# nemochina2008/soundgen_beta

Hardware: AMD Instinct MI355X
Metric: synthesized audio samples/sec (whole node) @44.1 kHz; RMS error vs R ref (higher is better)
Workload: dtype fp32 (fp64 phase); 1 GPU; C5: 65536 soundgen() calls drawn from the 33 presets (mixed sylLen and pitch contours), 44.1 kHz; calls=65536, calls_rank0=65536, samples=4311979595, parallelism=dp1 (one batch split by calls, LPT), plans_per_rank=6, failed_calls=0

## Files before the change

soundgen_beta_amd/csrc/sg_dev.h:

```cpp
#pragma once
#include <stdint.h>

struct SgSeg {
  double t0;
  double c0, c1, c2, c3, c4;
};

struct SgEpoch {
  int64_t w_off;
  int64_t amp_off;
  int64_t knot_off;
  int32_t seg_off;
  int32_t nseg;
  int32_t n;
  int32_t G;
  int32_t R;
  int32_t u0;
  double x1, xG;
  double xby;
  double invD;
  int32_t dj0, dj1;
  int64_t dk0;
  int32_t syl;
  int32_t pad;
// ... 131 lines not shown
  int32_t wl, M, nstages, fb;
  int32_t radix[SG_FFT_MAX_STAGES];
  int64_t tw;
  int64_t win;
  int32_t lds_bytes;
  int32_t kind;
  uint32_t mr_magic[SG_FFT_MAX_STAGES], ns_magic[SG_FFT_MAX_STAGES];
  uint32_t m_magic, hp_magic;
  int64_t tws;
};

constexpr int SG_FFT_WG = 0;
constexpr int SG_FFT_WAVE = 1;
constexpr int SG_FFT_DFT = 2;
constexpr int SG_FFT_ODD = 3;
constexpr int SG_WAVE_STATE = 24;
constexpr int SG_FFT_WAVES = 8;

#ifndef SG_NOISE_WAVES
#define SG_NOISE_WAVES 12
#endif
constexpr int SG_FFT_WAVES_NOISE = SG_NOISE_WAVES;
constexpr int sg_fft_waves(int phase) { return phase == 0 ? SG_FFT_WAVES_NOISE : SG_FFT_WAVES; }
constexpr int SG_PF_SRC = 20;
constexpr int SG_PF_PAIR = 10;

constexpr int SG_FRAME_FILTER = 0;
constexpr int SG_FRAME_NOISE = 1;
struct SgFrame {
  int64_t src;
// ... 156 lines not shown
```

soundgen_beta_amd/csrc/sg_exec.cpp:

```cpp
#include "sg_exec.h"
#include "sg_amp.h"
#include "sg_prof.h"

#include <algorithm>
#include <chrono>
#include <exception>
#include <thread>
#include <cmath>
#include <climits>
#include <atomic>
#include <map>
#include <cstdlib>
#include <cstdio>
#include <cstring>
#include <string>

namespace sg {

namespace {
#define HIPCHK(x)                                                                         \
  do {                                                                                    \
    hipError_t _e = (x);                                                                  \
    if (_e != hipSuccess)                                                                 \
      throw SgError(SG_E_DEVICE, std::string(#x) + ": " + hipGetErrorString(_e));     \
// ... 784 lines not shown
  DevicePlan& D0 = *runs[0].D;
  HIPCHK(hipEventRecord(D0.ev_fork, s));
  HIPCHK(hipStreamWaitEvent(s2, D0.ev_fork, 0));
  for (const PlanRun& r : runs) {
    device_execute_harm(*r.B, *r.D, r.out, s2, nullptr);
    HIPCHK(hipEventRecord(r.D->ev_join, s2));
  }
  for (const PlanRun& r : runs) device_execute_spec(*r.B, *r.D, r.out, s, nullptr, true, r.D->ev_join);
  HIPCHK(hipGetLastError());
}

void device_execute_spec(const Batch& B, const DevicePlan& D, float* d_out, hipStream_t s,
                         std::vector<SgProfEvent>* prof, bool join, hipEvent_t harm_done) {
  launch_spec_env(D, B, s);
  auto phase = [&](int ph) {
    const int64_t* r = B.fgroup_range[ph];
    const int64_t nseg = B.seg_range[ph][1] - B.seg_range[ph][0];
    hipEvent_t e0 = nullptr, e1 = nullptr;
    if (prof && nseg > 0) {
      HIPCHK(hipEventCreate(&e0));
      HIPCHK(hipEventCreate(&e1));
      HIPCHK(hipEventRecord(e0, s));
    }
    launch_stft_ola(D, ph, B.seg_range[ph][0], nseg, B.fgroup_lds[ph][0], s);
    if (prof && nseg > 0) {
      HIPCHK(hipEventRecord(e1, s));
      prof->push_back({SG_PROF_STFT_OLA, e0, e1});
    }
    launch_fft_frames(D, r[1], r[2] - r[1], B.fgroup_lds[ph][1], s);
    launch_fft_frames64(D, B, ph, s);
    const int64_t t0 = ph == 0 ? 0 : B.olatile_split, t1 = ph == 0 ? B.olatile_split : (int64_t)B.olatiles.size();
    const int64_t o0 = ph == 0 ? 0 : B.ola_split, o1 = ph == 0 ? B.ola_split : (int64_t)B.olas_dev.size();
    launch_ola(D, t0, t1 - t0, s);
    launch_ola_max(D, o0, o1 - o0, s);
  };
  phase(0);
  for (const Batch::Copy& c : B.copies)
    HIPCHK(hipMemcpyAsync(D.fs + c.fs_off, D.fl + c.fl_off, (size_t)c.n * sizeof(float), hipMemcpyDeviceToDevice, s));
  if (join) HIPCHK(hipStreamWaitEvent(s, harm_done, 0));
  launch_mix(D, 0, B.mixtile_hp, d_out, s);
  launch_mix_hp(D, B.mixtile_hp, B.mixtile_split - B.mixtile_hp, s);
  phase(1);
  launch_mix(D, B.mixtile_split, (int64_t)B.mixtiles.size() - B.mixtile_split, d_out, s);
  HIPCHK(hipGetLastError());
// ... 4 lines not shown
```

soundgen_beta_amd/csrc/sg_exec.h:

```cpp
#pragma once
#include <hip/hip_runtime.h>

#include <utility>
#include <vector>

#include "sg_plan.h"

namespace sg {

struct PcmJob {
  char* buf = nullptr;
  SgPcmCall* calls = nullptr;
  SgPcmTile* tiles = nullptr;
  SgPcmStat* stats = nullptr;
  int64_t n = 0, ntiles = 0;
  void prepare(const int64_t* off, const int64_t* len, int64_t n_calls, hipStream_t s);
  void run(const void* in, bool f64, int mode, double nrange, int16_t* out, hipStream_t s) const;
  void free();
};

struct DevicePlan {
  bool uploaded = false;
  char* arena = nullptr;
  size_t arena_bytes = 0;
// ... 88 lines not shown
void launch_ugather(const SgUJob* jobs, int64_t n_jobs, const float* us, float* fl, hipStream_t s);
void launch_sine_bank(const DevicePlan& D, int64_t k0, int64_t n, hipStream_t s);
void launch_sine_bank_pairs(const DevicePlan& D, int64_t k0, int64_t n, hipStream_t s);
void launch_sine_bank_tall(const DevicePlan& D, int64_t k0, int64_t n, hipStream_t s);
void launch_sine_bank_tall_pairs(const DevicePlan& D, int64_t k0, int64_t n, hipStream_t s);
void launch_syl_max(const DevicePlan& D, int64_t s0, int64_t n_syls, hipStream_t s);
void launch_piece_max(const DevicePlan& D, int64_t p0, int64_t n_ptiles, hipStream_t s);
void launch_harm_finalize(const DevicePlan& D, int64_t f0, int64_t n_stiles, float* out, hipStream_t s);
void launch_harm_copy(const DevicePlan& D, int64_t c0, int64_t n_ctiles, float* out, hipStream_t s);
void launch_sine_bank_hp(const DevicePlan& D, int64_t n, hipStream_t s);
void launch_sine_bank_tab(const DevicePlan& D, int logn, int64_t j0, int64_t n, float* out, hipStream_t s);
void launch_piece_max_hp(const DevicePlan& D, int64_t p0, int64_t n_ptiles, hipStream_t s);
void launch_harm_finalize_hp(const DevicePlan& D, int64_t n_stiles, hipStream_t s);
void launch_mix_hp(const DevicePlan& D, int64_t t0, int64_t n_tiles, hipStream_t s);
void launch_fft_frames64(const DevicePlan& D, const Batch& B, int ph, hipStream_t s);
void launch_fft_frames(const DevicePlan& D, int64_t g0, int64_t n_groups, int lds_bytes, hipStream_t s);
void launch_stft_ola(const DevicePlan& D, int phase, int64_t s0, int64_t n_segs, int lds_bytes, hipStream_t s);
void launch_ola(const DevicePlan& D, int64_t t0, int64_t n_tiles, hipStream_t s);
void launch_ola_max(const DevicePlan& D, int64_t o0, int64_t n_olas, hipStream_t s);
void launch_fft_probe(const SgFftGeom* geom, const float* fl, float* data, int M, int nframes, int inverse,
                      hipStream_t s);
void launch_mix(const DevicePlan& D, int64_t t0, int64_t n_tiles, float* out, hipStream_t s);
void launch_spec_env(const DevicePlan& D, const Batch& B, hipStream_t s);

}
```

soundgen_beta_amd/csrc/sg_fft.hip:

```cpp
#include <hip/hip_runtime.h>

#include <type_traits>

#include "sg_dev.h"
#include "sg_devfn.h"
#include "sg_fft64_dev.h"
#include "sg_roots.h"

namespace {

typedef float v2 __attribute__((ext_vector_type(2)));
__device__ __forceinline__ v2 V(float2 a) { return v2{a.x, a.y}; }
__device__ __forceinline__ float2 F(v2 a) { return make_float2(a.x, a.y); }
__device__ __forceinline__ v2 pfma(v2 a, v2 b, v2 c) { return __builtin_elementwise_fma(a, b, c); }
__device__ __forceinline__ v2 splat(float c) { return v2{c, c}; }
__device__ __forceinline__ v2 vmul(v2 a, v2 w) {
  v2 t, r;
  __asm__("v_pk_mul_f32 %0, %1, %2 op_sel_hi:[0,1]" : "=v"(t) : "v"(a), "v"(w));
  __asm__("v_pk_fma_f32 %0, %1, %2, %3 op_sel:[1,1,0] op_sel_hi:[1,0,1] neg_lo:[0,1,0]"
          : "=v"(r) : "v"(a), "v"(w), "v"(t));
  return r;
}
__device__ __forceinline__ v2 vmulc(v2 a, v2 w) {
  v2 t, r;
// ... 91 lines not shown
};

__device__ __forceinline__ void pack_pair(float2 yk, float2 ymk, float2 wNk, float2& zk, float2& zmk) {
  const float2 e = cadd(yk, cconj(ymk));
  const float2 d = csub(yk, cconj(ymk));
  const float2 o = cmulc(d, wNk);
  zk = make_float2(e.x - o.y, e.y + o.x);
  const float2 e2 = cadd(ymk, cconj(yk));
  const float2 d2 = csub(ymk, cconj(yk));
  const float2 o2 = make_float2(-(d2.x * wNk.x - d2.y * wNk.y), -(d2.x * wNk.y + d2.y * wNk.x));
  zmk = make_float2(e2.x - o2.y, e2.y + o2.x);
}

constexpr int SG_FFT_THREADS = 512;
constexpr int SG_FFT_SLOTS = 8192;

template <int R>
struct NbOf {
  static constexpr int value = (SG_FFT_SLOTS / SG_FFT_THREADS + R - 1) / R;
};

__device__ __forceinline__ int udiv(int n, uint32_t magic) {
  return magic ? (int)__umulhi((uint32_t)n, magic) : n;
}

template <int R, bool INV>
__device__ __forceinline__ void stage_ip(float2* X, int M, int Ns, const float2* twS, int fb, uint32_t mr_magic,
                                         uint32_t ns_magic) {
  constexpr int NB = NbOf<R>::value;
  constexpr bool ODD = (R % 2) == 1;
  constexpr int H = ODD ? (R - 1) / 2 : 1;
  const int MR = M / R;
  const int total = fb * MR;
  v2 st[NB][R];
  int base_o[NB];
  bool live[NB];
#pragma unroll
  for (int q = 0; q < NB; ++q) {
    const int idx = threadIdx.x + q * SG_FFT_THREADS;
    live[q] = idx < total;
    base_o[q] = 0;
    if (!live[q]) continue;
    const int f = udiv(idx, mr_magic);
    const int j = idx - f * MR;
    const float2* x = X + f * M;
    float2 v[R];
#pragma unroll
    for (int r = 0; r < R; ++r) v[r] = x[j + r * MR];
    const int jm = j - udiv(j, ns_magic) * Ns;
    if (Ns > 1) {
      const float2* tw = twS + (Ns - 1) + jm;
#pragma unroll
      for (int r = 1; r < R; ++r) {
        const float2 w = tw[(r - 1) * Ns];
// ... 27 lines not shown
#pragma unroll
      for (int k = 1; k <= H; ++k) {
        v2 a, b;
        odd_out<R, INV>(st[q], k, a, b);
        y[k * Ns] = F(a);
        y[(R - k) * Ns] = F(b);
      }
    } else {
#pragma unroll
      for (int r = 0; r < R; ++r) y[r * Ns] = F(st[q][r]);
    }
  }
  __syncthreads();
}

template <bool INV>
__device__ void fft_ip(float2* X, const SgFftGeom& g, const float2* twS, int fb) {
  int Ns = 1;
  for (int s = 0; s < g.nstages; ++s) {
    const int R = g.radix[s];
    const uint32_t mm = g.mr_magic[s], nm = g.ns_magic[s];
    int Ms = g.M;
    Ms = __builtin_amdgcn_readfirstlane(Ms);
    switch (R) {
#define SG_STAGE(RR) \
      case RR: stage_ip<RR, INV>(X, Ms, Ns, twS, fb, mm, nm); break;
      SG_STAGE(2) SG_STAGE(3) SG_STAGE(4) SG_STAGE(5) SG_STAGE(7) SG_STAGE(11) SG_STAGE(13) SG_STAGE(17)
      SG_STAGE(19) SG_STAGE(23) SG_STAGE(29) SG_STAGE(31)
#undef SG_STAGE
      default: break;
    }
    Ns *= R;
  }
}

__device__ __forceinline__ void sg_wave_fence() { __asm__ __volatile__("" ::: "memory"); }

template <int R>
struct NbW {
  static constexpr int value = SG_WAVE_STATE / R > 0 ? SG_WAVE_STATE / R : 1;
};
// ... 227 lines not shown
  }
  sg_wave_fence();
}

template <bool INV, int CM, int R0, int R1, int R2, bool MFMA = true, bool LAST = true>
__device__ __forceinline__ void fft_wc(float2* X, const float2* twS, const float4* A29, int lane SG_ST_PARAMS) {
  if constexpr (MFMA && CM == 1102 && R0 == 29) stage29_mfma<INV>(X, A29, lane);
  else stage_w<R0, INV, CM, 1>(X, CM, 1, twS, 0u, lane);
  SG_ST(INV ? 5 : 1);
  stage_w<R1, INV, CM, R0>(X, CM, R0, twS, 0u, lane);
  SG_ST(INV ? 6 : 2);
  if constexpr (LAST) stage_w<R2, INV, CM, R0 * R1>(X, CM, R0 * R1, twS, 0u, lane);
  SG_ST(INV ? 7 : 3);
}

template <bool INV>
__device__ void cdft(float2* X, const SgCdft& c, const SgFftGeom* __restrict__ geoms, const float* __restrict__ fl,
                     float2* Z, float2* tw) {
  const SgFftGeom& gs = geoms[c.geom];
  const int T = c.L ? c.L : c.n;
  const float2* twg = reinterpret_cast<const float2*>(fl + gs.tws);
  for (int t = threadIdx.x; t < T - 1; t += SG_FFT_THREADS) tw[t] = twg[t];
  if (!c.L) {
    __syncthreads();
    fft_ip<INV>(X, gs, tw, 1);
    return;
  }
  const int n = c.n, L = c.L;
  const float2* ch = reinterpret_cast<const float2*>(fl + c.chirp);
  const float2* bf = reinterpret_cast<const float2*>(fl + c.bf);
  for (int j = threadIdx.x; j < L; j += SG_FFT_THREADS)
    Z[j] = j < n ? cmul(INV ? cconj(X[j]) : X[j], ch[j]) : make_float2(0.f, 0.f);
  __syncthreads();
  fft_ip<false>(Z, gs, tw, 1);
  for (int k = threadIdx.x; k < L; k += SG_FFT_THREADS) Z[k] = cmul(Z[k], bf[k]);
  __syncthreads();
  fft_ip<true>(Z, gs, tw, 1);
  for (int k = threadIdx.x; k < n; k += SG_FFT_THREADS) {
    const float2 v = cmul(Z[k], ch[k]);
    X[k] = INV ? cconj(v) : v;
  }
  __syncthreads();
}

__device__ void odd_frame(const SgFrameGroup& G, const SgFrame* __restrict__ frames, const SgFftGeom& g,
                          const SgFftGeom* __restrict__ geoms, const float* __restrict__ fl, float* __restrict__ fs,
                          float4* lds4) {
  const int N = g.wl, M = g.M, N2 = 2 * M;
  const int T = max(g.cd[0].L ? g.cd[0].L : g.cd[0].n, g.cd[1].L ? g.cd[1].L : g.cd[1].n);
  float2* B = reinterpret_cast<float2*>(lds4);
  float2* Z = B + N;
  float2* tw = Z + T;
  const SgFrame F = frames[G.f0];
  const float* ham = fl + g.win;
  const float* han = ham + N;
  if (G.mode == SG_FRAME_FILTER) {
    const float* s = fs + F.src;
    for (int n = threadIdx.x; n < N; n += SG_FFT_THREADS) B[n] = make_float2(s[n] * ham[n], 0.f);
    __syncthreads();
    cdft<false>(B, g.cd[0], geoms, fl, Z, tw);
    const float* env = fl + F.env;
    const float invN = 1.f / (float)N;
    for (int k = threadIdx.x; k < M; k += SG_FFT_THREADS) {
      const float sc = invN * env[k];
      const float2 y = make_float2(B[k].x * sc, B[k].y * sc);
      B[k] = y;
      if (k > 0) B[N2 - k] = cconj(y);
      if (k == M - 1) B[M] = make_float2(y.x, 0.f);
    }
  } else {
    const float* u = fl + F.src;
    const float* flt = fl + F.env;
    for (int k = threadIdx.x; k < M; k += SG_FFT_THREADS) {
      const float2 y = make_float2(u[k] * flt[k], 0.f);
      B[k] = y;
      if (k > 0) B[N2 - k] = y;
      if (k == M - 1) B[M] = y;
    }
  }
  __syncthreads();
  cdft<true>(B, g.cd[1], geoms, fl, Z, tw);
  const float invN2 = 1.f / (float)N2;
  float* d = fs + F.dst;
  for (int i = threadIdx.x; i < N; i += SG_FFT_THREADS) d[i] = B[i < N2 ? i : i - N2].x * invN2 * han[i];
}

}

extern "C" __global__ __launch_bounds__(SG_FFT_THREADS) void sg_fft_frames(
    const SgFrameGroup* __restrict__ groups, const SgFrame* __restrict__ frames, const SgFftGeom* __restrict__ geoms,
    const float* __restrict__ fl, float* __restrict__ fs) {
  extern __shared__ float4 lds4[];
  float2* A = reinterpret_cast<float2*>(lds4);
  __shared__ SgFrame fr[16];
  const SgFrameGroup G = groups[blockIdx.x];
  const SgFftGeom& g = geoms[G.geom];
  if (g.kind == SG_FFT_ODD) {
    odd_frame(G, frames, g, geoms, fl, fs, lds4);
    return;
  }
  const int M = g.M, N = g.wl, fb = G.nf;
  const float2* twg = reinterpret_cast<const float2*>(fl + g.tw);
  const float2* twN = twg + M;
  float2* twM = A + fb * M;
  if (g.kind != SG_FFT_DFT) {
    const float2* tsg = reinterpret_cast<const float2*>(fl + g.tws);
    for (int t = threadIdx.x; t < M - 1; t += SG_FFT_THREADS) twM[t] = tsg[t];
  }
  if (threadIdx.x < fb) fr[threadIdx.x] = frames[G.f0 + threadIdx.x];
  __syncthreads();
  const float* ham = fl + g.win;
  const float* han = ham + N;
  const float invN = 1.f / (float)N;
  const int half = M / 2;
  const int npairs = fb * (half + 1);
  constexpr int NP = SG_FFT_SLOTS / 2 / SG_FFT_THREADS + 1;
  if (G.mode == SG_FRAME_FILTER) {
    for (int idx = threadIdx.x; idx < fb * M; idx += SG_FFT_THREADS) {
      const int f = udiv(idx, g.m_magic), n = idx - f * M;
      const float* s = fs + fr[f].src;
      A[idx] = make_float2(s[2 * n] * ham[2 * n], s[2 * n + 1] * ham[2 * n + 1]);
    }
    __syncthreads();
    if (g.kind == SG_FFT_DFT) cdft<false>(A, g.cd[0], geoms, fl, twM, twM + g.cd[0].L);
    else fft_ip<false>(A, g, twM, fb);
    float2 zk[NP], zm[NP], zh[NP];
    int pk[NP], pf[NP];
#pragma unroll
    for (int q = 0; q < NP; ++q) {
      const int idx = threadIdx.x + q * SG_FFT_THREADS;
      pk[q] = -1;
      if (idx >= npairs) continue;
      const int f = udiv(idx, g.hp_magic), k = idx - f * (half + 1);
      if (k != 0 && k >= M - k) continue;
      pk[q] = k;
      pf[q] = f;
      const float2* z = A + f * M;
      const float* env = fl + fr[f].env;
      auto X_at = [&](int kk) -> float2 {
        const float2 a = z[kk], b = z[(M - kk) % M];
        const float2 e = make_float2(0.5f * (a.x + b.x), 0.5f * (a.y - b.y));
        const float2 dd = make_float2(a.x - b.x, a.y + b.y);
        const float2 o = make_float2(0.5f * dd.y, -0.5f * dd.x);
        return cadd(e, cmul(o, twN[kk]));
      };
// ... 18 lines not shown
    __syncthreads();
#pragma unroll
    for (int q = 0; q < NP; ++q) {
      if (pk[q] < 0) continue;
      float2* out = A + pf[q] * M;
      const int k = pk[q];
      out[k] = zk[q];
      if (k == 0) {
        if (M % 2 == 0) out[half] = zh[q];
      } else {
        out[M - k] = zm[q];
      }
    }
    __syncthreads();
  } else {
    for (int idx = threadIdx.x; idx < npairs; idx += SG_FFT_THREADS) {
      const int f = udiv(idx, g.hp_magic), k = idx - f * (half + 1);
      const SgFrame& F = fr[f];
      const float* u = fl + F.src;
      const float* flt = fl + F.env;
      float2* out = A + f * M;
      if (k == 0) {
        const float y0 = u[0] * flt[0], nyq = u[M - 1] * flt[M - 1];
        out[0] = make_float2(y0 + nyq, y0 - nyq);
        if (M % 2 == 0) {
          const float2 yk = make_float2(u[half] * flt[half], 0.f);
          float2 a, b;
          pack_pair(yk, yk, twN[half], a, b);
          out[half] = a;
        }
      } else if (k < M - k) {
        const float2 yk = make_float2(u[k] * flt[k], 0.f), ym = make_float2(u[M - k] * flt[M - k], 0.f);
        float2 a, b;
        pack_pair(yk, ym, twN[k], a, b);
        out[k] = a;
        out[M - k] = b;
      }
    }
    __syncthreads();
  }
  if (g.kind == SG_FFT_DFT) cdft<true>(A, g.cd[0], geoms, fl, twM, twM + g.cd[0].L);
  else fft_ip<true>(A, g, twM, fb);
  for (int idx = threadIdx.x; idx < fb * M; idx += SG_FFT_THREADS) {
    const int f = udiv(idx, g.m_magic), n = idx - f * M;
    const float2 v = A[idx];
    float* d = fs + fr[f].dst;
    d[2 * n] = v.x * invN * han[2 * n];
    d[2 * n + 1] = v.y * invN * han[2 * n + 1];
  }
}

static_assert(SG_PF_PAIR <= SG_PF_SRC, "noise filter pairs alias the sound pairs");
struct FramePf {
  float2 s[SG_PF_SRC];
  float2 a[SG_PF_PAIR];
  float xh, xh2;
  __device__ __forceinline__ float2& b(int i) { return s[i]; }
  __device__ __forceinline__ const float2& b(int i) const { return s[i]; }
};

template <bool FUSED = false>
__device__ __forceinline__ void frame_prefetch(FramePf& P, const SgFrame& F, int mode, int M,
                                               const float* __restrict__ fl, const float* __restrict__ fs, int lane) {
  const int half = M / 2;
// ... 1037 lines not shown
  } while (0)

static void lds_opt_in(const void* fn, int lds_bytes, const char* name) {
  static std::mutex mu;
  static std::map<std::pair<const void*, int>, int> done;
  int dev = 0;
  if (hipGetDevice(&dev) != hipSuccess) throw SgError(SG_E_DEVICE, std::string(name) + ": hipGetDevice failed");
  std::lock_guard<std::mutex> lk(mu);
  int& have = done[{fn, dev}];
  if (lds_bytes <= have) return;
  if (hipFuncSetAttribute(fn, hipFuncAttributeMaxDynamicSharedMemorySize, lds_bytes) != hipSuccess)
    throw SgError(SG_E_DEVICE, std::string(name) + ": dynamic LDS " + std::to_string(lds_bytes) + " B refused");
  have = lds_bytes;
}

void launch_fft_frames(const DevicePlan& D, int64_t g0, int64_t n_groups, int lds_bytes, hipStream_t s) {
  if (n_groups <= 0) return;
  lds_opt_in(reinterpret_cast<const void*>(&sg_fft_frames), lds_bytes, "sg_fft_frames");
  hipLaunchKernelGGL(sg_fft_frames, dim3((unsigned)n_groups), dim3(SG_FFT_THREADS), lds_bytes, s, D.fgroups + g0,
                     D.frames,
                     D.geoms, D.fl, D.fs);
  SG_LAUNCHED("sg_fft_frames");
}
void launch_stft_ola(const DevicePlan& D, int phase, int64_t s0, int64_t n_segs, int lds_bytes, hipStream_t s) {
  if (n_segs <= 0) return;
  auto* k = phase == 0 ? &sg_stft_ola_noise : &sg_stft_ola;
  lds_opt_in(reinterpret_cast<const void*>(k), lds_bytes, phase == 0 ? "sg_stft_ola_noise" : "sg_stft_ola");
  const int W = sg_fft_waves(phase);
  if (n_segs % W) throw SgError(SG_E_DEVICE, "sg_stft_ola: segment count not a multiple of the workgroup's waves");
  hipLaunchKernelGGL(k, dim3((unsigned)(n_segs / W)), dim3(W * 64), lds_bytes, s,
                     D.olasegs + s0,
                     D.olas, D.frames, D.geoms, D.fl, D.fs, D.olatilemax);
// ... 74 lines not shown
```

soundgen_beta_amd/csrc/sg_plan.h:

```cpp
#pragma once
#include <cstdint>
#include <functional>
#include <memory>
#include <utility>
#include <vector>

#include "sg_dev.h"
#include "sg_rmath.h"
#include "soundgen_hip.h"

namespace sg {

template <class T>
struct NoInitAlloc : std::allocator<T> {
  template <class U>
  struct rebind { using other = NoInitAlloc<U>; };
  NoInitAlloc() = default;
  template <class U>
  NoInitAlloc(const NoInitAlloc<U>&) noexcept {}
  T* allocate(size_t n) {
    if (n * sizeof(T) < SG_BULK_HUGE) return std::allocator<T>::allocate(n);
    return static_cast<T*>(bulk_alloc(n * sizeof(T)));
  }
  void deallocate(T* p, size_t n) noexcept {
// ... 75 lines not shown
  std::vector<SgOla> olas[2];
  std::vector<SgFrame64> frames64;
  std::vector<int32_t> roots64_wl;
  std::vector<int64_t> roots64_off, frames64_tab;
  int64_t roots64_total = 0;
  int32_t frames64_maxwl = 0;
  int64_t frames64_noise = 0;
  int64_t frames64_w[2] = {0, 0};
  std::vector<SgNoiseItem> items;
  std::vector<SgMix> mixes[2];
  struct Copy { int64_t fl_off, fs_off, n; };
  std::vector<Copy> copies;
  std::vector<SgFrameGroup> fgroups;
  int64_t fgroup_range[2][3] = {{0, 0, 0}, {0, 0, 0}};
  int fgroup_lds[2][2] = {{0, 0}, {0, 0}};
  std::vector<SgOla> olas_dev;
  std::vector<SgOlaTile> olatiles;
  int64_t olatile_split = 0, ola_split = 0;
  std::vector<SgSegment> olasegs;
  int32_t n_segslots = 0;
  int64_t seg_range[2][2] = {{0, 0}, {0, 0}};
  std::vector<SgMix> mixes_dev;
  std::vector<SgMixTile> mixtiles;
  int64_t mixtile_split = 0;
  int64_t mixtile_hp = 0;
  bulk<double> cknots;
  int64_t w_total = 0;
  int64_t w64_total = 0;
  int64_t fh_total = 0;
  int64_t hp_bouts = 0;
// ... 91 lines not shown
```

soundgen_beta_amd/csrc/sg_plan_spec.cpp:

```cpp
#include <algorithm>
#include <atomic>
#include <cmath>
#include <complex>
#include <cstdio>
#include <cstdlib>
#include <cstring>
#include <map>
#include <memory>
#include <mutex>
#include <string>

#include "sg_plan.h"
#include "sg_prof.h"

#ifndef SG_SEG_SORT
#define SG_SEG_SORT 1
#endif
#ifndef SG_ENV_SORT
#define SG_ENV_SORT 1
#endif

namespace sg {

namespace {
// ... 116 lines not shown
      if (m > 0) b[L - m] = b[m];
    }
    dft_smooth(b, bf);
    vec v(2 * (size_t)L);
    for (int k = 0; k < L; ++k) {
      v[2 * k] = bf[k].real() / L;
      v[2 * k + 1] = bf[k].imag() / L;
    }
    return v;
  });
  c.chirp = fl_push(B, ch->data(), (int64_t)ch->size());
  c.bf = fl_push(B, bv->data(), (int64_t)bv->size());
  return c;
}
static int cdft_size(const SgCdft& c) { return c.L ? c.L : c.n; }

static int geometry_odd(Batch& B, int wl) {
  SgFftGeom g{};
  g.wl = wl;
  g.M = wl / 2;
  g.kind = SG_FFT_ODD;
  g.fb = 1;
  g.cd[0] = make_cdft(B, wl);
  g.cd[1] = make_cdft(B, 2 * g.M);
  const int T = std::max(cdft_size(g.cd[0]), cdft_size(g.cd[1]));
  g.lds_bytes = (int32_t)(((int64_t)wl + 2 * (int64_t)T) * 8);
  if (g.lds_bytes > 160 * 1024) throw SgError(SG_E_UNSUPPORTED, "FFT: odd window length exceeds the LDS budget");
  g.win = push_windows(B, wl);
  for (size_t i = 0; i < B.geoms.size(); ++i)
    if (B.geoms[i].wl == wl) return (int)i;
  B.geoms.push_back(g);
  return (int)B.geoms.size() - 1;
}

int geometry(Batch& B, int wl) {
  for (size_t i = 0; i < B.geoms.size(); ++i)
    if (B.geoms[i].wl == wl) return (int)i;
// ... 51 lines not shown
    });
    g.tws = fl_push(B, ts->data(), (int64_t)ts->size());
  }
  g.win = push_windows(B, wl);
  g.kind = dft ? SG_FFT_DFT : SG_FFT_WAVE;
  for (int s = 0; s < g.nstages && !dft; ++s) {
    const int r = g.radix[s], nb = (g.M / r + 63) / 64;
    if (nb > std::max(1, SG_WAVE_STATE / r)) g.kind = SG_FFT_WG;
  }
  if (!dft && (g.M > 64 * SG_PF_SRC || g.M / 2 + 1 > 64 * SG_PF_PAIR)) g.kind = SG_FFT_WG;
  if (!dft && (int64_t)(SG_FFT_WAVES + 4) * g.M * 8 > 160 * 1024) g.kind = SG_FFT_WG;
  if (g.kind == SG_FFT_WAVE) {
    g.fb = SG_FFT_WAVES;
    g.lds_bytes = (SG_FFT_WAVES + 4) * g.M * 8;
  } else if (g.kind == SG_FFT_DFT) {
    g.fb = 1;
    g.lds_bytes = (g.M + 2 * g.cd[0].L) * 8;
    if (g.lds_bytes > 160 * 1024) throw SgError(SG_E_UNSUPPORTED, "FFT: Bluestein frame exceeds the LDS budget");
  } else {
    g.fb = std::max(1, std::min(16, kFftSlots / g.M));
    if (g.fb * g.M > kFftSlots) throw SgError(SG_E_UNSUPPORTED, "FFT: window too long for LDS (wl > 16384)");
    g.lds_bytes = (g.fb + 1) * g.M * 8;
  }
  auto magic = [](int d) -> uint32_t { return d <= 1 ? 0u : (uint32_t)(((1ull << 32) + (uint64_t)d - 1) / (uint64_t)d); };
  int ns = 1;
  for (int s = 0; s < g.nstages; ++s) {
    g.mr_magic[s] = magic(g.M / g.radix[s]);
    g.ns_magic[s] = magic(ns);
    ns *= g.radix[s];
  }
  g.m_magic = magic(g.M);
// ... 552 lines not shown
      for (size_t w = i; w < i + 4 && w < B.envtasks.size(); ++w) { mx = std::max(mx, cost(B.envtasks[w])); wsum += cost(B.envtasks[w]); }
      wmax += 4 * mx;
    }
    std::fprintf(stderr, "sg plan: envelope tasks %zu, workgroup cost %.3g, used %.3g (%.1f%% idle)\n", B.envtasks.size(), wmax,
                 wsum, wmax > 0 ? 100.0 * (wmax - wsum) / wmax : 0.0);
  }
  B.fgroups.clear();
  std::vector<int64_t> pos[2];
  for (int ph = 0; ph < 2; ++ph) {
    const size_t ng = B.geoms.size();
    std::vector<int64_t> rank(ng), start(ng + 1, 0);
    {
      std::vector<int32_t> og(ng);
      for (size_t g = 0; g < ng; ++g) og[g] = (int32_t)g;
      std::stable_sort(og.begin(), og.end(), [&](int32_t a, int32_t b) {
        const int ka = B.geoms[a].kind == SG_FFT_WAVE ? 0 : 1, kb = B.geoms[b].kind == SG_FFT_WAVE ? 0 : 1;
        return ka != kb ? ka < kb : a < b;
      });
      for (size_t r = 0; r < ng; ++r) rank[og[r]] = (int64_t)r;
    }
    for (int32_t gi : B.frame_geom[ph]) ++start[rank[gi] + 1];
    for (size_t r = 0; r < ng; ++r) start[r + 1] += start[r];
    std::vector<int64_t> idx(B.frames[ph].size());
    for (size_t i = 0; i < idx.size(); ++i) idx[start[rank[B.frame_geom[ph][i]]]++] = (int64_t)i;
    std::vector<SgFrame> fr(idx.size());
    std::vector<int32_t> fg(idx.size());
    pos[ph].assign(idx.size(), 0);
    for (size_t i = 0; i < idx.size(); ++i) {
      fr[i] = B.frames[ph][idx[i]];
      fg[i] = B.frame_geom[ph][idx[i]];
      pos[ph][idx[i]] = (int64_t)i;
    }
    B.frames[ph] = fr;
    B.frame_geom[ph] = fg;
    const int32_t base = ph == 0 ? 0 : (int32_t)B.frames[0].size();
    B.fgroup_lds[ph][0] = B.fgroup_lds[ph][1] = 0;
    B.fgroup_range[ph][0] = B.fgroup_range[ph][1] = (int64_t)B.fgroups.size();
    for (size_t i = 0; i < fr.size();) {
      const int gi = fg[i];
      const SgFftGeom& g = B.geoms[gi];
      if (g.kind == SG_FFT_WAVE) {
        B.fgroup_lds[ph][0] = std::max(B.fgroup_lds[ph][0], (sg_fft_waves(ph) + 4) * g.M * 8 + (g.M == 1102 ? 2048 : 0));
        ++i;
        continue;
      }
      size_t j = i;
      while (j < fr.size() && fg[j] == gi && (int)(j - i) < g.fb) ++j;
      B.fgroups.push_back(SgFrameGroup{gi, ph == 0 ? SG_FRAME_NOISE : SG_FRAME_FILTER, base + (int32_t)i,
                                       (int32_t)(j - i)});
      B.fgroup_lds[ph][1] = std::max(B.fgroup_lds[ph][1], g.lds_bytes);
      i = j;
    }
    B.fgroup_range[ph][2] = (int64_t)B.fgroups.size();
  }
  B.olas_dev.clear();
  B.olatiles.clear();
  B.olasegs.clear();
  B.ola_split = (int64_t)B.olas[0].size();
  for (int ph = 0; ph < 2; ++ph) {
    if (ph == 1) B.olatile_split = (int64_t)B.olatiles.size();
    const int32_t base = ph == 0 ? 0 : (int32_t)B.frames[0].size();
    for (const SgOla& o0 : B.olas[ph]) {
      SgOla o = o0;
      if (o0.fidx >= 0) o.fidx = base + (int32_t)pos[ph][o0.fidx];
      const int32_t oi = (int32_t)B.olas_dev.size();
      if (!o.fused) {
        o.tile0 = (int32_t)B.olatiles.size();
        for (int64_t q0 = 0; q0 < o.len; q0 += SG_OLA_TILE) B.olatiles.push_back(SgOlaTile{oi, 0, q0});
// ... 143 lines not shown
      const SgFftGeom& g = B.geoms[gs[i].second];
      std::string rs;
      for (int s = 0; s < g.nstages; ++s) rs += (s ? "x" : "") + std::to_string(g.radix[s]);
      std::fprintf(stderr, "sg plan: geom wl=%d M=%d radices %s: %lld frames\n", g.wl, g.M, rs.c_str(),
                   (long long)gs[i].first);
    }
    std::map<int32_t, int64_t> gun;
    for (const SgFrameGroup& fg : B.fgroups) gun[fg.geom] += fg.nf;
    for (const auto& kv : gun) {
      const SgFftGeom& g = B.geoms[kv.first];
      std::string rs;
      for (int s = 0; s < g.nstages; ++s) rs += (s ? "x" : "") + std::to_string(g.radix[s]);
      std::fprintf(stderr, "sg plan: unfused geom wl=%d M=%d kind %d radices %s: %lld frames\n", g.wl, g.M, g.kind,
                   rs.c_str(), (long long)kv.second);
    }
    std::fprintf(stderr, "sg plan: %lld fused segments (%lld slots incl. padding), %lld frames owned, %lld computed (%.1f%% recomputed)\n",
                 (long long)real, (long long)B.olasegs.size(), (long long)owned, (long long)run,
                 owned ? 100.0 * (double)(run - owned) / (double)owned : 0.0);
  }
  for (SgNoiseItem& it : B.items)
    if (it.flags & SG_ITEM_FILTER_OLA) {
      it.ola += (int32_t)B.ola_split;
      it.flags &= ~SG_ITEM_FILTER_OLA;
    }
  B.mixes_dev.clear();
  B.mixtiles.clear();
  for (int pass = 0; pass < 3; ++pass) {
    const int ph = pass == 2 ? 1 : 0;
    if (pass == 1) B.mixtile_hp = (int64_t)B.mixtiles.size();
    if (pass == 2) B.mixtile_split = (int64_t)B.mixtiles.size();
// ... 19 lines not shown
```

Before: 14.01 billion samples/s.

## Split unfused FFT frame launches into LDS size classes with a smaller-slot kernel

Unfused FFT frame groups are sorted and split into three classes by geometry kind, transform size, largest radix and LDS footprint. Bluestein and odd-length geometries that fit the smaller slot count and radix cap go to a new kernel variant. That variant is built with fewer per-thread slots, a waves-per-EU hint and only radices up to 13, and each class launches with its own LDS size. The aim is lower register and LDS pressure, so more blocks fit per CU for small frames, and less twiddle restaging through a per-geometry cache. The code also allows several sequential frames per group for DFT and odd kinds (default 1), and the extra launches add overhead.

```diff
diff --git a/soundgen_beta_amd/csrc/sg_dev.h b/soundgen_beta_amd/csrc/sg_dev.h
--- a/soundgen_beta_amd/csrc/sg_dev.h
+++ b/soundgen_beta_amd/csrc/sg_dev.h
@@ -169,6 +169,20 @@
 constexpr int SG_FFT_WAVE = 1;
 constexpr int SG_FFT_DFT = 2;
 constexpr int SG_FFT_ODD = 3;
+constexpr int SG_FRAMES_S_SLOTS = 4608;
+#ifndef SG_FRAMES_S_MAXR
+#define SG_FRAMES_S_MAXR 13
+#endif
+constexpr int SG_FRAMES_MAX_FB = 16;
+#ifndef SG_FRAMES_FB
+#define SG_FRAMES_FB 1
+#endif
+static_assert(SG_FRAMES_FB >= 1 && SG_FRAMES_FB <= SG_FRAMES_MAX_FB, "frames per group");
+#ifndef SG_FRAMES_CLASSES
+#define SG_FRAMES_CLASSES 1
+#endif
+constexpr int SG_FRAMES_NCLASS = 3;
+constexpr int SG_FRAMES_LDS_CLASS[SG_FRAMES_NCLASS - 1] = {80000, 160 * 1024};
 constexpr int SG_WAVE_STATE = 24;
 constexpr int SG_FFT_WAVES = 8;
 
diff --git a/soundgen_beta_amd/csrc/sg_exec.cpp b/soundgen_beta_amd/csrc/sg_exec.cpp
--- a/soundgen_beta_amd/csrc/sg_exec.cpp
+++ b/soundgen_beta_amd/csrc/sg_exec.cpp
@@ -822,7 +822,6 @@
                          std::vector<SgProfEvent>* prof, bool join, hipEvent_t harm_done) {
   launch_spec_env(D, B, s);
   auto phase = [&](int ph) {
-    const int64_t* r = B.fgroup_range[ph];
     const int64_t nseg = B.seg_range[ph][1] - B.seg_range[ph][0];
     hipEvent_t e0 = nullptr, e1 = nullptr;
     if (prof && nseg > 0) {
@@ -835,7 +834,9 @@
       HIPCHK(hipEventRecord(e1, s));
       prof->push_back({SG_PROF_STFT_OLA, e0, e1});
     }
-    launch_fft_frames(D, r[1], r[2] - r[1], B.fgroup_lds[ph][1], s);
+    for (int c = 0; c < SG_FRAMES_NCLASS; ++c)
+      launch_fft_frames(D, B.fgroup_cls[ph][c], B.fgroup_cls[ph][c + 1] - B.fgroup_cls[ph][c], B.fgroup_cls_lds[ph][c],
+                        c < SG_FRAMES_NCLASS - 1, s);
     launch_fft_frames64(D, B, ph, s);
     const int64_t t0 = ph == 0 ? 0 : B.olatile_split, t1 = ph == 0 ? B.olatile_split : (int64_t)B.olatiles.size();
     const int64_t o0 = ph == 0 ? 0 : B.ola_split, o1 = ph == 0 ? B.ola_split : (int64_t)B.olas_dev.size();
diff --git a/soundgen_beta_amd/csrc/sg_exec.h b/soundgen_beta_amd/csrc/sg_exec.h
--- a/soundgen_beta_amd/csrc/sg_exec.h
+++ b/soundgen_beta_amd/csrc/sg_exec.h
@@ -126,7 +126,7 @@
 void launch_harm_finalize_hp(const DevicePlan& D, int64_t n_stiles, hipStream_t s);
 void launch_mix_hp(const DevicePlan& D, int64_t t0, int64_t n_tiles, hipStream_t s);
 void launch_fft_frames64(const DevicePlan& D, const Batch& B, int ph, hipStream_t s);
-void launch_fft_frames(const DevicePlan& D, int64_t g0, int64_t n_groups, int lds_bytes, hipStream_t s);
+void launch_fft_frames(const DevicePlan& D, int64_t g0, int64_t n_groups, int lds_bytes, bool small, hipStream_t s);
 void launch_stft_ola(const DevicePlan& D, int phase, int64_t s0, int64_t n_segs, int lds_bytes, hipStream_t s);
 void launch_ola(const DevicePlan& D, int64_t t0, int64_t n_tiles, hipStream_t s);
 void launch_ola_max(const DevicePlan& D, int64_t o0, int64_t n_olas, hipStream_t s);
diff --git a/soundgen_beta_amd/csrc/sg_fft.hip b/soundgen_beta_amd/csrc/sg_fft.hip
--- a/soundgen_beta_amd/csrc/sg_fft.hip
+++ b/soundgen_beta_amd/csrc/sg_fft.hip
@@ -129,20 +129,26 @@
 
 constexpr int SG_FFT_THREADS = 512;
 constexpr int SG_FFT_SLOTS = 8192;
-
-template <int R>
+#ifndef SG_FRAMES_S_THREADS
+#define SG_FRAMES_S_THREADS 512
+#endif
+#ifndef SG_FRAMES_S_WPE
+#define SG_FRAMES_S_WPE 4
+#endif
+
+template <int R, int TH, int SL>
 struct NbOf {
-  static constexpr int value = (SG_FFT_SLOTS / SG_FFT_THREADS + R - 1) / R;
+  static constexpr int value = ((SL + TH - 1) / TH + R - 1) / R;
 };
 
 __device__ __forceinline__ int udiv(int n, uint32_t magic) {
   return magic ? (int)__umulhi((uint32_t)n, magic) : n;
 }
 
-template <int R, bool INV>
+template <int R, bool INV, int TH, int SL>
 __device__ __forceinline__ void stage_ip(float2* X, int M, int Ns, const float2* twS, int fb, uint32_t mr_magic,
                                          uint32_t ns_magic) {
-  constexpr int NB = NbOf<R>::value;
+  constexpr int NB = NbOf<R, TH, SL>::value;
   constexpr bool ODD = (R % 2) == 1;
   constexpr int H = ODD ? (R - 1) / 2 : 1;
   const int MR = M / R;
@@ -152,7 +158,7 @@
   bool live[NB];
 #pragma unroll
   for (int q = 0; q < NB; ++q) {
-    const int idx = threadIdx.x + q * SG_FFT_THREADS;
+    const int idx = threadIdx.x + q * TH;
     live[q] = idx < total;
     base_o[q] = 0;
     if (!live[q]) continue;
@@ -210,8 +216,9 @@
   __syncthreads();
 }
 
-template <bool INV>
+template <bool INV, int TH, int SL>
 __device__ void fft_ip(float2* X, const SgFftGeom& g, const float2* twS, int fb) {
+  constexpr int MAXR = SL == SG_FRAMES_S_SLOTS ? SG_FRAMES_S_MAXR : 31;
   int Ns = 1;
   for (int s = 0; s < g.nstages; ++s) {
     const int R = g.radix[s];
@@ -220,7 +227,7 @@
     Ms = __builtin_amdgcn_readfirstlane(Ms);
     switch (R) {
 #define SG_STAGE(RR) \
-      case RR: stage_ip<RR, INV>(X, Ms, Ns, twS, fb, mm, nm); break;
+      case RR: if constexpr (RR <= MAXR) stage_ip<RR, INV, TH, SL>(X, Ms, Ns, twS, fb, mm, nm); break;
       SG_STAGE(2) SG_STAGE(3) SG_STAGE(4) SG_STAGE(5) SG_STAGE(7) SG_STAGE(11) SG_STAGE(13) SG_STAGE(17)
       SG_STAGE(19) SG_STAGE(23) SG_STAGE(29) SG_STAGE(31)
 #undef SG_STAGE
@@ -478,121 +485,111 @@
   SG_ST(INV ? 7 : 3);
 }
 
-template <bool INV>
+template <bool INV, int TH, int SL>
 __device__ void cdft(float2* X, const SgCdft& c, const SgFftGeom* __restrict__ geoms, const float* __restrict__ fl,
-                     float2* Z, float2* tw) {
+                     float2* Z, float2* tw, int& staged) {
   const SgFftGeom& gs = geoms[c.geom];
   const int T = c.L ? c.L : c.n;
-  const float2* twg = reinterpret_cast<const float2*>(fl + gs.tws);
-  for (int t = threadIdx.x; t < T - 1; t += SG_FFT_THREADS) tw[t] = twg[t];
+  if (staged != c.geom) {
+    const float2* twg = reinterpret_cast<const float2*>(fl + gs.tws);
+    for (int t = threadIdx.x; t < T - 1; t += TH) tw[t] = twg[t];
+    staged = c.geom;
+  }
   if (!c.L) {
     __syncthreads();
-    fft_ip<INV>(X, gs, tw, 1);
+    fft_ip<INV, TH, SL>(X, gs, tw, 1);
     return;
   }
   const int n = c.n, L = c.L;
   const float2* ch = reinterpret_cast<const float2*>(fl + c.chirp);
   const float2* bf = reinterpret_cast<const float2*>(fl + c.bf);
-  for (int j = threadIdx.x; j < L; j += SG_FFT_THREADS)
+  for (int j = threadIdx.x; j < L; j += TH)
     Z[j] = j < n ? cmul(INV ? cconj(X[j]) : X[j], ch[j]) : make_float2(0.f, 0.f);
   __syncthreads();
-  fft_ip<false>(Z, gs, tw, 1);
-  for (int k = threadIdx.x; k < L; k += SG_FFT_THREADS) Z[k] = cmul(Z[k], bf[k]);
+  fft_ip<false, TH, SL>(Z, gs, tw, 1);
+  for (int k = threadIdx.x; k < L; k += TH) Z[k] = cmul(Z[k], bf[k]);
   __syncthreads();
-  fft_ip<true>(Z, gs, tw, 1);
-  for (int k = threadIdx.x; k < n; k += SG_FFT_THREADS) {
+  fft_ip<true, TH, SL>(Z, gs, tw, 1);
+  for (int k = threadIdx.x; k < n; k += TH) {
     const float2 v = cmul(Z[k], ch[k]);
     X[k] = INV ? cconj(v) : v;
   }
   __syncthreads();
 }
 
-__device__ void odd_frame(const SgFrameGroup& G, const SgFrame* __restrict__ frames, const SgFftGeom& g,
-                          const SgFftGeom* __restrict__ geoms, const float* __restrict__ fl, float* __restrict__ fs,
-                          float4* lds4) {
+template <int TH, int SL>
+__device__ void odd_frames(const SgFrameGroup& G, const SgFrame* __restrict__ frames, const SgFftGeom& g,
+                           const SgFftGeom* __restrict__ geoms, const float* __restrict__ fl, float* __restrict__ fs,
+                           float4* lds4) {
   const int N = g.wl, M = g.M, N2 = 2 * M;
   const int T = max(g.cd[0].L ? g.cd[0].L : g.cd[0].n, g.cd[1].L ? g.cd[1].L : g.cd[1].n);
   float2* B = reinterpret_cast<float2*>(lds4);
   float2* Z = B + N;
   float2* tw = Z + T;
-  const SgFrame F = frames[G.f0];
   const float* ham = fl + g.win;
   const float* han = ham + N;
-  if (G.mode == SG_FRAME_FILTER) {
-    const float* s = fs + F.src;
-    for (int n = threadIdx.x; n < N; n += SG_FFT_THREADS) B[n] = make_float2(s[n] * ham[n], 0.f);
+  int staged = -1;
+  for (int it = 0; it < G.nf; ++it) {
+    if (it) __syncthreads();
+    const SgFrame F = frames[G.f0 + it];
+    if (G.mode == SG_FRAME_FILTER) {
+      const float* s = fs + F.src;
+      for (int n = threadIdx.x; n < N; n += TH) B[n] = make_float2(s[n] * ham[n], 0.f);
+      __syncthreads();
+      cdft<false, TH, SL>(B, g.cd[0], geoms, fl, Z, tw, staged);
+      const float* env = fl + F.env;
+      const float invN = 1.f / (float)N;
+      for (int k = threadIdx.x; k < M; k += TH) {
+        const float sc = invN * env[k];
+        const float2 y = make_float2(B[k].x * sc, B[k].y * sc);
+        B[k] = y;
+        if (k > 0) B[N2 - k] = cconj(y);
+        if (k == M - 1) B[M] = make_float2(y.x, 0.f);
+      }
+    } else {
+      const float* u = fl + F.src;
+      const float* flt = fl + F.env;
+      for (int k = threadIdx.x; k < M; k += TH) {
+        const float2 y = make_float2(u[k] * flt[k], 0.f);
+        B[k] = y;
+        if (k > 0) B[N2 - k] = y;
+        if (k == M - 1) B[M] = y;
+      }
+    }
     __syncthreads();
-    cdft<false>(B, g.cd[0], geoms, fl, Z, tw);
-    const float* env = fl + F.env;
-    const float invN = 1.f / (float)N;
-    for (int k = threadIdx.x; k < M; k += SG_FFT_THREADS) {
-      const float sc = invN * env[k];
-      const float2 y = make_float2(B[k].x * sc, B[k].y * sc);
-      B[k] = y;
-      if (k > 0) B[N2 - k] = cconj(y);
-      if (k == M - 1) B[M] = make_float2(y.x, 0.f);
-    }
-  } else {
-    const float* u = fl + F.src;
-    const float* flt = fl + F.env;
-    for (int k = threadIdx.x; k < M; k += SG_FFT_THREADS) {
-      const float2 y = make_float2(u[k] * flt[k], 0.f);
-      B[k] = y;
-      if (k > 0) B[N2 - k] = y;
-      if (k == M - 1) B[M] = y;
-    }
-  }
-  __syncthreads();
-  cdft<true>(B, g.cd[1], geoms, fl, Z, tw);
-  const float invN2 = 1.f / (float)N2;
-  float* d = fs + F.dst;
-  for (int i = threadIdx.x; i < N; i += SG_FFT_THREADS) d[i] = B[i < N2 ? i : i - N2].x * invN2 * han[i];
-}
-
-}
-
-extern "C" __global__ __launch_bounds__(SG_FFT_THREADS) void sg_fft_frames(
-    const SgFrameGroup* __restrict__ groups, const SgFrame* __restrict__ frames, const SgFftGeom* __restrict__ geoms,
-    const float* __restrict__ fl, float* __restrict__ fs) {
-  extern __shared__ float4 lds4[];
-  float2* A = reinterpret_cast<float2*>(lds4);
-  __shared__ SgFrame fr[16];
-  const SgFrameGroup G = groups[blockIdx.x];
-  const SgFftGeom& g = geoms[G.geom];
-  if (g.kind == SG_FFT_ODD) {
-    odd_frame(G, frames, g, geoms, fl, fs, lds4);
-    return;
-  }
-  const int M = g.M, N = g.wl, fb = G.nf;
-  const float2* twg = reinterpret_cast<const float2*>(fl + g.tw);
-  const float2* twN = twg + M;
-  float2* twM = A + fb * M;
-  if (g.kind != SG_FFT_DFT) {
-    const float2* tsg = reinterpret_cast<const float2*>(fl + g.tws);
-    for (int t = threadIdx.x; t < M - 1; t += SG_FFT_THREADS) twM[t] = tsg[t];
-  }
-  if (threadIdx.x < fb) fr[threadIdx.x] = frames[G.f0 + threadIdx.x];
-  __syncthreads();
+    cdft<true, TH, SL>(B, g.cd[1], geoms, fl, Z, tw, staged);
+    const float invN2 = 1.f / (float)N2;
+    float* d = fs + F.dst;
+    for (int i = threadIdx.x; i < N; i += TH) d[i] = B[i < N2 ? i : i - N2].x * invN2 * han[i];
+  }
+}
+
+template <int TH, int SL>
+__device__ __forceinline__ void even_frames(int mode, const SgFftGeom& g, const SgFftGeom* __restrict__ geoms,
+                                            const float* __restrict__ fl, float* __restrict__ fs, float2* A,
+                                            float2* twM, const SgFrame* fr, int fb, int& staged) {
+  const int M = g.M, N = g.wl;
+  const float2* twN = reinterpret_cast<const float2*>(fl + g.tw) + M;
   const float* ham = fl + g.win;
   const float* han = ham + N;
   const float invN = 1.f / (float)N;
   const int half = M / 2;
   const int npairs = fb * (half + 1);
-  constexpr int NP = SG_FFT_SLOTS / 2 / SG_FFT_THREADS + 1;
-  if (G.mode == SG_FRAME_FILTER) {
-    for (int idx = threadIdx.x; idx < fb * M; idx += SG_FFT_THREADS) {
+  constexpr int NP = SL / 2 / TH + 1;
+  if (mode == SG_FRAME_FILTER) {
+    for (int idx = threadIdx.x; idx < fb * M; idx += TH) {
       const int f = udiv(idx, g.m_magic), n = idx - f * M;
       const float* s = fs + fr[f].src;
       A[idx] = make_float2(s[2 * n] * ham[2 * n], s[2 * n + 1] * ham[2 * n + 1]);
     }
     __syncthreads();
-    if (g.kind == SG_FFT_DFT) cdft<false>(A, g.cd[0], geoms, fl, twM, twM + g.cd[0].L);
-    else fft_ip<false>(A, g, twM, fb);
+    if (g.kind == SG_FFT_DFT) cdft<false, TH, SL>(A, g.cd[0], geoms, fl, twM, twM + g.cd[0].L, staged);
+    else fft_ip<false, TH, SL>(A, g, twM, fb);
     float2 zk[NP], zm[NP], zh[NP];
     int pk[NP], pf[NP];
 #pragma unroll
     for (int q = 0; q < NP; ++q) {
-      const int idx = threadIdx.x + q * SG_FFT_THREADS;
+      const int idx = threadIdx.x + q * TH;
       pk[q] = -1;
       if (idx >= npairs) continue;
       const int f = udiv(idx, g.hp_magic), k = idx - f * (half + 1);
@@ -641,7 +638,7 @@
     }
     __syncthreads();
   } else {
-    for (int idx = threadIdx.x; idx < npairs; idx += SG_FFT_THREADS) {
+    for (int idx = threadIdx.x; idx < npairs; idx += TH) {
       const int f = udiv(idx, g.hp_magic), k = idx - f * (half + 1);
       const SgFrame& F = fr[f];
       const float* u = fl + F.src;
@@ -666,15 +663,63 @@
     }
     __syncthreads();
   }
-  if (g.kind == SG_FFT_DFT) cdft<true>(A, g.cd[0], geoms, fl, twM, twM + g.cd[0].L);
-  else fft_ip<true>(A, g, twM, fb);
-  for (int idx = threadIdx.x; idx < fb * M; idx += SG_FFT_THREADS) {
+  if (g.kind == SG_FFT_DFT) cdft<true, TH, SL>(A, g.cd[0], geoms, fl, twM, twM + g.cd[0].L, staged);
+  else fft_ip<true, TH, SL>(A, g, twM, fb);
+  for (int idx = threadIdx.x; idx < fb * M; idx += TH) {
     const int f = udiv(idx, g.m_magic), n = idx - f * M;
     const float2 v = A[idx];
     float* d = fs + fr[f].dst;
     d[2 * n] = v.x * invN * han[2 * n];
     d[2 * n + 1] = v.y * invN * han[2 * n + 1];
   }
+}
+
+template <int TH, int SL>
+__device__ __forceinline__ void frame_group(const SgFrameGroup& G, const SgFrame* __restrict__ frames,
+                                            const SgFftGeom* __restrict__ geoms, const float* __restrict__ fl,
+                                            float* __restrict__ fs, float4* lds4, SgFrame* fr) {
+  float2* A = reinterpret_cast<float2*>(lds4);
+  const SgFftGeom& g = geoms[G.geom];
+  if (g.kind == SG_FFT_ODD) {
+    odd_frames<TH, SL>(G, frames, g, geoms, fl, fs, lds4);
+    return;
+  }
+  const int M = g.M;
+  const bool dft = g.kind == SG_FFT_DFT;
+  const int fb = dft ? 1 : G.nf;
+  float2* twM = A + fb * M;
+  if (!dft) {
+    const float2* tsg = reinterpret_cast<const float2*>(fl + g.tws);
+    for (int t = threadIdx.x; t < M - 1; t += TH) twM[t] = tsg[t];
+  }
+  if (threadIdx.x < G.nf) fr[threadIdx.x] = frames[G.f0 + threadIdx.x];
+  __syncthreads();
+  int staged = -1;
+  if (!dft) {
+    even_frames<TH, SL>(G.mode, g, geoms, fl, fs, A, twM, fr, fb, staged);
+    return;
+  }
+  for (int it = 0; it < G.nf; ++it) {
+    if (it) __syncthreads();
+    even_frames<TH, SL>(G.mode, g, geoms, fl, fs, A, twM, fr + it, 1, staged);
+  }
+}
+
+}
+
+extern "C" __global__ __launch_bounds__(SG_FFT_THREADS) void sg_fft_frames(
+    const SgFrameGroup* __restrict__ groups, const SgFrame* __restrict__ frames, const SgFftGeom* __restrict__ geoms,
+    const float* __restrict__ fl, float* __restrict__ fs) {
+  extern __shared__ float4 lds4[];
+  __shared__ SgFrame fr[SG_FRAMES_MAX_FB];
+  frame_group<SG_FFT_THREADS, SG_FFT_SLOTS>(groups[blockIdx.x], frames, geoms, fl, fs, lds4, fr);
+}
+extern "C" __global__ __launch_bounds__(SG_FRAMES_S_THREADS) __attribute__((amdgpu_waves_per_eu(SG_FRAMES_S_WPE, 8))) void
+sg_fft_frames_s(const SgFrameGroup* __restrict__ groups, const SgFrame* __restrict__ frames,
+                const SgFftGeom* __restrict__ geoms, const float* __restrict__ fl, float* __restrict__ fs) {
+  extern __shared__ float4 lds4[];
+  __shared__ SgFrame fr[SG_FRAMES_MAX_FB];
+  frame_group<SG_FRAMES_S_THREADS, SG_FRAMES_S_SLOTS>(groups[blockIdx.x], frames, geoms, fl, fs, lds4, fr);
 }
 
 static_assert(SG_PF_PAIR <= SG_PF_SRC, "noise filter pairs alias the sound pairs");
@@ -1742,8 +1787,15 @@
   have = lds_bytes;
 }
 
-void launch_fft_frames(const DevicePlan& D, int64_t g0, int64_t n_groups, int lds_bytes, hipStream_t s) {
+void launch_fft_frames(const DevicePlan& D, int64_t g0, int64_t n_groups, int lds_bytes, bool small, hipStream_t s) {
   if (n_groups <= 0) return;
+  if (small) {
+    lds_opt_in(reinterpret_cast<const void*>(&sg_fft_frames_s), lds_bytes, "sg_fft_frames_s");
+    hipLaunchKernelGGL(sg_fft_frames_s, dim3((unsigned)n_groups), dim3(SG_FRAMES_S_THREADS), lds_bytes, s,
+                       D.fgroups + g0, D.frames, D.geoms, D.fl, D.fs);
+    SG_LAUNCHED("sg_fft_frames_s");
+    return;
+  }
   lds_opt_in(reinterpret_cast<const void*>(&sg_fft_frames), lds_bytes, "sg_fft_frames");
   hipLaunchKernelGGL(sg_fft_frames, dim3((unsigned)n_groups), dim3(SG_FFT_THREADS), lds_bytes, s, D.fgroups + g0,
                      D.frames,
diff --git a/soundgen_beta_amd/csrc/sg_plan.h b/soundgen_beta_amd/csrc/sg_plan.h
--- a/soundgen_beta_amd/csrc/sg_plan.h
+++ b/soundgen_beta_amd/csrc/sg_plan.h
@@ -113,6 +113,8 @@
   std::vector<SgFrameGroup> fgroups;
   int64_t fgroup_range[2][3] = {{0, 0, 0}, {0, 0, 0}};
   int fgroup_lds[2][2] = {{0, 0}, {0, 0}};
+  int64_t fgroup_cls[2][SG_FRAMES_NCLASS + 1] = {};
+  int fgroup_cls_lds[2][SG_FRAMES_NCLASS] = {};
   std::vector<SgOla> olas_dev;
   std::vector<SgOlaTile> olatiles;
   int64_t olatile_split = 0, ola_split = 0;
diff --git a/soundgen_beta_amd/csrc/sg_plan_spec.cpp b/soundgen_beta_amd/csrc/sg_plan_spec.cpp
--- a/soundgen_beta_amd/csrc/sg_plan_spec.cpp
+++ b/soundgen_beta_amd/csrc/sg_plan_spec.cpp
@@ -154,13 +154,27 @@
   return c;
 }
 static int cdft_size(const SgCdft& c) { return c.L ? c.L : c.n; }
+constexpr int kSeqFb = SG_FRAMES_CLASSES ? SG_FRAMES_FB : 1;
+static int frames_class(const Batch& B, const SgFftGeom& g) {
+  if (!SG_FRAMES_CLASSES || (g.kind != SG_FFT_DFT && g.kind != SG_FFT_ODD)) return SG_FRAMES_NCLASS - 1;
+  const int T = g.kind == SG_FFT_DFT ? cdft_size(g.cd[0]) : std::max(cdft_size(g.cd[0]), cdft_size(g.cd[1]));
+  if (T > SG_FRAMES_S_SLOTS) return SG_FRAMES_NCLASS - 1;
+  for (int i = 0; i < (g.kind == SG_FFT_DFT ? 1 : 2); ++i) {
+    const SgFftGeom& gs = B.geoms[(size_t)g.cd[i].geom];
+    for (int s = 0; s < gs.nstages; ++s)
+      if (gs.radix[s] > SG_FRAMES_S_MAXR) return SG_FRAMES_NCLASS - 1;
+  }
+  for (int c = 0; c < SG_FRAMES_NCLASS - 1; ++c)
+    if (g.lds_bytes <= SG_FRAMES_LDS_CLASS[c]) return c;
+  return SG_FRAMES_NCLASS - 1;
+}
 
 static int geometry_odd(Batch& B, int wl) {
   SgFftGeom g{};
   g.wl = wl;
   g.M = wl / 2;
   g.kind = SG_FFT_ODD;
-  g.fb = 1;
+  g.fb = kSeqFb;
   g.cd[0] = make_cdft(B, wl);
   g.cd[1] = make_cdft(B, 2 * g.M);
   const int T = std::max(cdft_size(g.cd[0]), cdft_size(g.cd[1]));
@@ -242,7 +256,7 @@
     g.fb = SG_FFT_WAVES;
     g.lds_bytes = (SG_FFT_WAVES + 4) * g.M * 8;
   } else if (g.kind == SG_FFT_DFT) {
-    g.fb = 1;
+    g.fb = kSeqFb;
     g.lds_bytes = (g.M + 2 * g.cd[0].L) * 8;
     if (g.lds_bytes > 160 * 1024) throw SgError(SG_E_UNSUPPORTED, "FFT: Bluestein frame exceeds the LDS budget");
   } else {
@@ -825,8 +839,12 @@
       std::vector<int32_t> og(ng);
       for (size_t g = 0; g < ng; ++g) og[g] = (int32_t)g;
       std::stable_sort(og.begin(), og.end(), [&](int32_t a, int32_t b) {
-        const int ka = B.geoms[a].kind == SG_FFT_WAVE ? 0 : 1, kb = B.geoms[b].kind == SG_FFT_WAVE ? 0 : 1;
-        return ka != kb ? ka < kb : a < b;
+        const int ka = B.geoms[a].kind == SG_FFT_WAVE ? -1 : frames_class(B, B.geoms[a]);
+        const int kb = B.geoms[b].kind == SG_FFT_WAVE ? -1 : frames_class(B, B.geoms[b]);
+        if (ka != kb) return ka < kb;
+        if (SG_FRAMES_CLASSES && ka >= 0 && B.geoms[a].lds_bytes != B.geoms[b].lds_bytes)
+          return B.geoms[a].lds_bytes > B.geoms[b].lds_bytes;
+        return a < b;
       });
       for (size_t r = 0; r < ng; ++r) rank[og[r]] = (int64_t)r;
     }
@@ -847,6 +865,10 @@
     const int32_t base = ph == 0 ? 0 : (int32_t)B.frames[0].size();
     B.fgroup_lds[ph][0] = B.fgroup_lds[ph][1] = 0;
     B.fgroup_range[ph][0] = B.fgroup_range[ph][1] = (int64_t)B.fgroups.size();
+    for (int c = 0; c < SG_FRAMES_NCLASS; ++c) {
+      B.fgroup_cls[ph][c] = -1;
+      B.fgroup_cls_lds[ph][c] = 0;
+    }
     for (size_t i = 0; i < fr.size();) {
       const int gi = fg[i];
       const SgFftGeom& g = B.geoms[gi];
@@ -860,9 +882,14 @@
       B.fgroups.push_back(SgFrameGroup{gi, ph == 0 ? SG_FRAME_NOISE : SG_FRAME_FILTER, base + (int32_t)i,
                                        (int32_t)(j - i)});
       B.fgroup_lds[ph][1] = std::max(B.fgroup_lds[ph][1], g.lds_bytes);
+      const int c = frames_class(B, g);
+      if (B.fgroup_cls[ph][c] < 0) B.fgroup_cls[ph][c] = (int64_t)B.fgroups.size() - 1;
+      B.fgroup_cls_lds[ph][c] = std::max(B.fgroup_cls_lds[ph][c], g.lds_bytes);
       i = j;
     }
-    B.fgroup_range[ph][2] = (int64_t)B.fgroups.size();
+    B.fgroup_range[ph][2] = B.fgroup_cls[ph][SG_FRAMES_NCLASS] = (int64_t)B.fgroups.size();
+    for (int c = SG_FRAMES_NCLASS - 1; c >= 0; --c)
+      if (B.fgroup_cls[ph][c] < 0) B.fgroup_cls[ph][c] = B.fgroup_cls[ph][c + 1];
   }
   B.olas_dev.clear();
   B.olatiles.clear();
@@ -1036,6 +1063,28 @@
       std::fprintf(stderr, "sg plan: unfused geom wl=%d M=%d kind %d radices %s: %lld frames\n", g.wl, g.M, g.kind,
                    rs.c_str(), (long long)kv.second);
     }
+    for (int ph = 0; ph < 2; ++ph) {
+      int64_t nfr[4] = {}, ngr[4] = {}, nol[4] = {}, cfr[SG_FRAMES_NCLASS] = {}, cgr[SG_FRAMES_NCLASS] = {};
+      for (int64_t i = B.fgroup_range[ph][1]; i < B.fgroup_range[ph][2]; ++i) {
+        const SgFrameGroup& fg = B.fgroups[(size_t)i];
+        const SgFftGeom& g = B.geoms[fg.geom];
+        nfr[g.kind & 3] += fg.nf;
+        ++ngr[g.kind & 3];
+        cfr[frames_class(B, g)] += fg.nf;
+        ++cgr[frames_class(B, g)];
+      }
+      const int32_t fbase = ph == 0 ? 0 : (int32_t)B.frames[0].size();
+      const size_t o_lo = ph == 0 ? 0 : (size_t)B.ola_split, o_hi = ph == 0 ? (size_t)B.ola_split : B.olas_dev.size();
+      for (size_t oi = o_lo; oi < o_hi; ++oi)
+        if (!B.olas_dev[oi].fused && B.olas_dev[oi].fidx >= 0)
+          ++nol[B.geoms[B.frame_geom[ph][B.olas_dev[oi].fidx - fbase]].kind & 3];
+      for (int k : {SG_FFT_WG, SG_FFT_DFT, SG_FFT_ODD})
+        std::fprintf(stderr, "sg plan: phase %d unfused kind %d: %lld frames, %lld groups, %lld OLAs\n", ph, k,
+                     (long long)nfr[k], (long long)ngr[k], (long long)nol[k]);
+      for (int c = 0; c < SG_FRAMES_NCLASS; ++c)
+        std::fprintf(stderr, "sg plan: phase %d unfused launch class %d: %lld frames, %lld groups, LDS %d B\n", ph, c,
+                     (long long)cfr[c], (long long)cgr[c], B.fgroup_cls_lds[ph][c]);
+    }
     std::fprintf(stderr, "sg plan: %lld fused segments (%lld slots incl. padding), %lld frames owned, %lld computed (%.1f%% recomputed)\n",
                  (long long)real, (long long)B.olasegs.size(), (long long)owned, (long long)run,
                  owned ? 100.0 * (double)(run - owned) / (double)owned : 0.0);
```

Result: no change. 13.99 billion samples/s, median of 2 (-0.1%).
